# fanzhongyi/diffusion

Hardware: AMD Instinct MI355X
Metric: U-Net training images/sec @256 (SD-2-base U-Net, precomputed latents 4x32x32) (higher is better)
Workload: dtype bf16; 1 GPU; SD-2-base U-Net train step, latents 4x32x32, text 77x1024, batch 256/GPU (global 256), microbatch 256, AdamW, dp1; global_batch=256, microbatch=256, parallelism=dp1, params=865910724

## Files before the change

diffusion_amd/csrc/attention.hip:

```cpp
#include <type_traits>

#include "common.hpp"
#include "attn_lds.hpp"
#include "diffusion_amd.h"

namespace {

struct AttnParams {
  const bf16 *Q, *K, *V, *O, *dO;
  bf16 *Out, *dQ, *dK, *dV;
  float *L2, *Delta;
  long ldq, ldk, ldv, ldo, lddo, lddq, lddk, lddv;
  int B, H, Nq, Nk;
  float sc;
  float scale;
};

#ifdef DA_STAMPS
__device__ unsigned long long* g_attn_stamp_buf;
__device__ int g_attn_stamp_wgs;
#define ASTAMP(v) v = __builtin_amdgcn_s_memtime()
#else
#define ASTAMP(v) do {} while (0)
#endif

typedef float f32x2 __attribute__((ext_vector_type(2)));
DEVINL f32x2 pair(const f32x16& v, int i) { return f32x2{v[2 * i], v[2 * i + 1]}; }
DEVINL void set_pair(f32x16& v, int i, f32x2 x) { v[2 * i] = x.x; v[2 * i + 1] = x.y; }
DEVINL f32x2 fma2(f32x2 a, f32x2 b, f32x2 c) {
  float x = fmaf(a.x, b.x, c.x), y = fmaf(a.y, b.y, c.y);
  asm("" : "+v"(x));
  asm("" : "+v"(y));
  return f32x2{x, y};
}
DEVINL f32x2 mul2(f32x2 a, f32x2 b) {
  float x = a.x * b.x, y = a.y * b.y;
  asm("" : "+v"(x));
  asm("" : "+v"(y));
  return f32x2{x, y};
}
DEVINL f32x2 add2(f32x2 a, f32x2 b) {
  float x = a.x + b.x, y = a.y + b.y;
  asm("" : "+v"(x));
  asm("" : "+v"(y));
  return f32x2{x, y};
}
DEVINL f32x2 exp2_2(f32x2 x) { return f32x2{__builtin_amdgcn_exp2f(x.x), __builtin_amdgcn_exp2f(x.y)}; }

DEVINL float max3(float a, float b, float c) {
  float r;
  asm("v_max3_f32 %0, %1, %2, %3" : "=v"(r) : "v"(a), "v"(b), "v"(c));
  return r;
}

DEVINL void xcd_block_id(int& blk, int& hd, int& b) {
  const int nb = gridDim.x, nh = gridDim.y;
  const int total = nb * nh * gridDim.z;
  const int w = blockIdx.x + nb * (blockIdx.y + nh * blockIdx.z);
  const int q = total >> 3, r = total & 7;
// ... 8 lines not shown
__device__ __attribute__((aligned(256))) unsigned char g_attn_zero[256];
DEVINL void dma4(const void* g, char* l) {
  __builtin_amdgcn_global_load_lds((const __attribute__((address_space(1))) void*)g,
                                   (__attribute__((address_space(3))) void*)l, 4, 0, 0);
}

constexpr int FW_STAGE = 64 * 128 + 64 * TR_LD;

template <bool CAUSAL>
__global__ __launch_bounds__(256) void attn_fwd_kernel(AttnParams p) {
  extern __shared__ __attribute__((aligned(16))) char smem[];
  const int tid = threadIdx.x, lane = tid & 63;
  const int wave = __builtin_amdgcn_readfirstlane(tid >> 6);
  const int h = lane >> 5, r = lane & 31;
  int blk, hd, b;
  xcd_block_id(blk, hd, b);
  const int q = blk * 128 + wave * 32 + r;
  const bool qv = q < p.Nq;

  bf16x8 qf[4];
#pragma unroll
  for (int ks = 0; ks < 4; ++ks)
    qf[ks] = qv ? ld8(p.Q + ((long)b * p.Nq + q) * p.ldq + hd * 64 + ks * 16 + h * 8) : zero8();

  f32x16 o0, o1;
#pragma unroll
  for (int i = 0; i < 16; ++i) { o0[i] = 0.f; o1[i] = 0.f; }
  float m = -INFINITY, l = 0.f;

  const int nk_eff = CAUSAL ? min(p.Nk, blk * 128 + 128) : p.Nk;
  const int nt = (nk_eff + 63) / 64;
  const int drow = wave * 8 + (lane >> 3), pc = lane & 7;
  const int lc = (pc ^ swz_key(drow)) * 8;
  const bf16* kp = p.K + ((long)b * p.Nk + drow) * p.ldk + hd * 64;
  const bf16* vp = p.V + ((long)b * p.Nk + drow) * p.ldv + hd * 64;
  const char* zero = reinterpret_cast<const char*>(g_attn_zero);
  auto dma = [&](int t, int st) {
    char* S = smem + st * FW_STAGE + wave * 1024;
#pragma unroll
    for (int i = 0; i < 2; ++i) {
      const bool ok = t * 64 + drow + 32 * i < p.Nk;
      dma16(ok ? (const void*)(kp + 32 * i * p.ldk + lc) : (const void*)zero, S + i * 4096);
      dma16(ok ? (const void*)(vp + 32 * i * p.ldv + lc) : (const void*)zero, S + 8192 + i * 4096);
    }
    kp += 64 * p.ldk;
    vp += 64 * p.ldv;
  };
  auto sync_tile = [&]() {
    asm volatile("s_waitcnt vmcnt(0)" ::: "memory");
    __builtin_amdgcn_s_barrier();
    asm volatile("" ::: "memory");
  };

  dma(0, 0);
  sync_tile();
  auto step = [&](int t, auto tail_tag) {
    constexpr bool TAIL = decltype(tail_tag)::value;
    if (t + 1 < nt) dma(t + 1, (t + 1) & 1);
    const char* Ks = smem + (t & 1) * FW_STAGE;
    const char* Vs = Ks + 64 * 128;
    f32x16 s0, s1;
#pragma unroll
    for (int i = 0; i < 16; ++i) { s0[i] = 0.f; s1[i] = 0.f; }
#pragma unroll
    for (int ks = 0; ks < 4; ++ks) {
      bf16x8 k0 = *reinterpret_cast<const bf16x8*>(Ks + swz128(r, 2 * ks + h));
      bf16x8 k1 = *reinterpret_cast<const bf16x8*>(Ks + swz128(32 + r, 2 * ks + h));
      s0 = __builtin_amdgcn_mfma_f32_32x32x16_bf16(k0, qf[ks], s0, 0, 0, 0);
      s1 = __builtin_amdgcn_mfma_f32_32x32x16_bf16(k1, qf[ks], s1, 0, 0, 0);
    }
    short4v tv[2][4][2];
    const unsigned vto = lds_offset(Vs);
#pragma unroll
    for (int s2 = 0; s2 < 2; ++s2) {
      tr_frag_issue(vto, 16 * s2, 0, lane, tv[s2][0][0], tv[s2][0][1]);
      tr_frag_issue(vto, 16 * s2, 32, lane, tv[s2][1][0], tv[s2][1][1]);
      tr_frag_issue(vto, 32 + 16 * s2, 0, lane, tv[s2][2][0], tv[s2][2][1]);
      tr_frag_issue(vto, 32 + 16 * s2, 32, lane, tv[s2][3][0], tv[s2][3][1]);
    }
    if constexpr (TAIL) {
      const int klim = CAUSAL ? min(p.Nk, q + 1) : p.Nk;
#pragma unroll
      for (int i = 0; i < 16; ++i) {
        int key = t * 64 + acc_row(i, lane);
        if (key >= klim) s0[i] = -INFINITY;
        if (key + 32 >= klim) s1[i] = -INFINITY;
      }
    }
    float mx = fmaxf(s0[0], s1[0]);
#pragma unroll
    for (int i = 1; i < 16; ++i) mx = max3(mx, s0[i], s1[i]);
    mx = fmaxf(mx, xor32(mx));
    if (__any(mx > m)) {
      const float mn = fmaxf(m, mx);
      const float alpha = __builtin_amdgcn_exp2f((m - mn) * p.sc);
      l *= alpha;
      const f32x2 al2 = {alpha, alpha};
#pragma unroll
      for (int i = 0; i < 8; ++i) {
        set_pair(o0, i, mul2(pair(o0, i), al2));
        set_pair(o1, i, mul2(pair(o1, i), al2));
      }
      m = mn;
    }
    const float msc = -m * p.sc;
    const f32x2 sc2 = {p.sc, p.sc}, msc2 = {msc, msc};
    f32x2 ls2 = {0.f, 0.f};
#pragma unroll
    for (int i = 0; i < 8; ++i) {
      const f32x2 e0 = exp2_2(fma2(pair(s0, i), sc2, msc2));
      const f32x2 e1 = exp2_2(fma2(pair(s1, i), sc2, msc2));
      set_pair(s0, i, e0);
      set_pair(s1, i, e1);
      ls2 = add2(ls2, add2(e0, e1));
    }
    l += ls2.x + ls2.y;
    lds_wait_for<0>(tv[0][0][0], tv[0][0][1], tv[0][1][0], tv[0][1][1], tv[0][2][0], tv[0][2][1], tv[0][3][0], tv[0][3][1],
                    tv[1][0][0], tv[1][0][1], tv[1][1][0], tv[1][1][1], tv[1][2][0], tv[1][2][1], tv[1][3][0], tv[1][3][1]);
#pragma unroll
    for (int s2 = 0; s2 < 2; ++s2) {
      bf16x8 pa = pack8(s0, s2), pb = pack8(s1, s2);
      o0 = __builtin_amdgcn_mfma_f32_32x32x16_bf16(tr_frag_join(tv[s2][0][0], tv[s2][0][1]), pa, o0, 0, 0, 0);
      o1 = __builtin_amdgcn_mfma_f32_32x32x16_bf16(tr_frag_join(tv[s2][1][0], tv[s2][1][1]), pa, o1, 0, 0, 0);
      o0 = __builtin_amdgcn_mfma_f32_32x32x16_bf16(tr_frag_join(tv[s2][2][0], tv[s2][2][1]), pb, o0, 0, 0, 0);
      o1 = __builtin_amdgcn_mfma_f32_32x32x16_bf16(tr_frag_join(tv[s2][3][0], tv[s2][3][1]), pb, o1, 0, 0, 0);
    }
    sync_tile();
  };
  if constexpr (CAUSAL) {
    for (int t = 0; t < nt; ++t) step(t, std::true_type{});
  } else {
    const int nfull = p.Nk / 64;
    for (int t = 0; t < nfull; ++t) step(t, std::false_type{});
    if (nfull < nt) step(nfull, std::true_type{});
  }
  const float lt = l + xor32(l);
  const float inv = 1.0f / lt;
  if (qv) {
    bf16* op = p.Out + ((long)b * p.Nq + q) * p.ldo + hd * 64;
#pragma unroll
    for (int rg = 0; rg < 4; ++rg) {
      bf16x4 a, c;
#pragma unroll
      for (int e = 0; e < 4; ++e) {
        a[e] = f2bf(o0[rg * 4 + e] * inv);
        c[e] = f2bf(o1[rg * 4 + e] * inv);
      }
      *reinterpret_cast<bf16x4*>(op + 8 * rg + 4 * h) = a;
      *reinterpret_cast<bf16x4*>(op + 32 + 8 * rg + 4 * h) = c;
    }
    if (h == 0) p.L2[((long)b * p.H + hd) * p.Nq + q] = m * p.sc + log2f(lt);
  }
}

constexpr int DQ_STAGE = 2 * 64 * 128;

__global__ __launch_bounds__(256, 3) void attn_bwd_dq_kernel(AttnParams p) {
  extern __shared__ __attribute__((aligned(16))) char smem[];
  const int tid = threadIdx.x, lane = tid & 63;
  const int wave = __builtin_amdgcn_readfirstlane(tid >> 6);
  const int h = lane >> 5, r = lane & 31;
  int blk, hd, b;
  xcd_block_id(blk, hd, b);
  const int q = blk * 128 + wave * 32 + r;
  const bool qv = q < p.Nq;

  bf16x8 qf[4], dof[4];
  float delta = 0.f;
#pragma unroll
  for (int ks = 0; ks < 4; ++ks) {
    const int c = hd * 64 + ks * 16 + h * 8;
    qf[ks] = qv ? ld8(p.Q + ((long)b * p.Nq + q) * p.ldq + c) : zero8();
    dof[ks] = qv ? ld8(p.dO + ((long)b * p.Nq + q) * p.lddo + c) : zero8();
    bf16x8 of = qv ? ld8(p.O + ((long)b * p.Nq + q) * p.ldo + c) : zero8();
#pragma unroll
    for (int j = 0; j < 8; ++j) delta += bf2f(dof[ks][j]) * bf2f(of[j]);
  }
  delta += xor32(delta);
  const long statidx = ((long)b * p.H + hd) * p.Nq + q;
  const float nL2q = qv ? -p.L2[statidx] : 0.f;
  if (qv && h == 0) p.Delta[statidx] = delta;

  f32x16 d0, d1;
#pragma unroll
  for (int i = 0; i < 16; ++i) { d0[i] = 0.f; d1[i] = 0.f; }

  const int nt = (p.Nk + 63) / 64;
  const int drow = wave * 8 + (lane >> 3), pc = lane & 7;
  const int lc = (pc ^ swz_key(drow)) * 8;
  const bf16* kp = p.K + ((long)b * p.Nk + drow) * p.ldk + hd * 64;
  const bf16* vp = p.V + ((long)b * p.Nk + drow) * p.ldv + hd * 64;
  const char* zero = reinterpret_cast<const char*>(g_attn_zero);
  auto dma = [&](int t, int st) {
    char* S = smem + st * DQ_STAGE + wave * 1024;
#pragma unroll
    for (int i = 0; i < 2; ++i) {
      const bool ok = t * 64 + drow + 32 * i < p.Nk;
      dma16(ok ? (const void*)(kp + 32 * i * p.ldk + lc) : (const void*)zero, S + i * 4096);
      dma16(ok ? (const void*)(vp + 32 * i * p.ldv + lc) : (const void*)zero, S + 8192 + i * 4096);
    }
    kp += 64 * p.ldk;
    vp += 64 * p.ldv;
  };
  auto sync_tile = [&]() {
    asm volatile("s_waitcnt vmcnt(0)" ::: "memory");
    __builtin_amdgcn_s_barrier();
    asm volatile("" ::: "memory");
  };

  dma(0, 0);
  sync_tile();
  auto step = [&](int t, auto tail_tag) {
    constexpr bool TAIL = decltype(tail_tag)::value;
    if (t + 1 < nt) dma(t + 1, (t + 1) & 1);
    const char* Ks = smem + (t & 1) * DQ_STAGE;
    const char* Vs = Ks + 64 * 128;
    const char* Kt = Ks;
#pragma unroll
    for (int half = 0; half < 2; ++half) {
      const int kb = half * 32;
      if (TAIL && t * 64 + kb >= p.Nk) break;
      f32x16 s, dp;
#pragma unroll
      for (int i = 0; i < 16; ++i) { s[i] = 0.f; dp[i] = -delta; }
#pragma unroll
      for (int ks = 0; ks < 4; ++ks) {
        bf16x8 kf = *reinterpret_cast<const bf16x8*>(Ks + swz128(kb + r, 2 * ks + h));
        bf16x8 vf = *reinterpret_cast<const bf16x8*>(Vs + swz128(kb + r, 2 * ks + h));
        s = __builtin_amdgcn_mfma_f32_32x32x16_bf16(kf, qf[ks], s, 0, 0, 0);
        dp = __builtin_amdgcn_mfma_f32_32x32x16_bf16(vf, dof[ks], dp, 0, 0, 0);
      }
      short4v tk0[2][2], tk1[2][2];
      const unsigned kto = lds_offset(Kt);
#pragma unroll
      for (int s2 = 0; s2 < 2; ++s2) {
        tr_frag_issue(kto, kb + 16 * s2, 0, lane, tk0[s2][0], tk0[s2][1]);
        tr_frag_issue(kto, kb + 16 * s2, 32, lane, tk1[s2][0], tk1[s2][1]);
      }
      {
        const f32x2 sc2 = {p.sc, p.sc}, nl2 = {nL2q, nL2q};
#pragma unroll
        for (int i = 0; i < 8; ++i) {
          const f32x2 pv = exp2_2(__builtin_elementwise_fma(pair(s, i), sc2, nl2));
          set_pair(s, i, pv * pair(dp, i));
        }
      }
      if constexpr (TAIL) {
#pragma unroll
        for (int i = 0; i < 16; ++i)
          if (t * 64 + kb + acc_row(i, lane) >= p.Nk) s[i] = 0.f;
      }
      bf16x8 dsf[2] = {pack8(s, 0), pack8(s, 1)};
      lds_wait_for<0>(tk0[0][0], tk0[0][1], tk1[0][0], tk1[0][1], tk0[1][0], tk0[1][1], tk1[1][0], tk1[1][1]);
#pragma unroll
      for (int s2 = 0; s2 < 2; ++s2) {
        d0 = __builtin_amdgcn_mfma_f32_32x32x16_bf16(tr_frag_join(tk0[s2][0], tk0[s2][1]), dsf[s2], d0, 0, 0, 0);
        d1 = __builtin_amdgcn_mfma_f32_32x32x16_bf16(tr_frag_join(tk1[s2][0], tk1[s2][1]), dsf[s2], d1, 0, 0, 0);
      }
    }
    sync_tile();
  };
  const int nfull = p.Nk / 64;
  for (int t = 0; t < nfull; ++t) step(t, std::false_type{});
  if (nfull < nt) step(nfull, std::true_type{});
  if (qv) {
    bf16* op = p.dQ + ((long)b * p.Nq + q) * p.lddq + hd * 64;
#pragma unroll
    for (int rg = 0; rg < 4; ++rg) {
      bf16x4 a, c;
#pragma unroll
      for (int e = 0; e < 4; ++e) {
        a[e] = f2bf(d0[rg * 4 + e] * p.scale);
        c[e] = f2bf(d1[rg * 4 + e] * p.scale);
      }
      *reinterpret_cast<bf16x4*>(op + 8 * rg + 4 * h) = a;
      *reinterpret_cast<bf16x4*>(op + 32 + 8 * rg + 4 * h) = c;
    }
  }
}

constexpr int kv_stage(int QT) { return 2 * QT * 128 + 2 * QT * 4; }

template <int KV_QT>
__global__ __launch_bounds__(256, 2) void attn_bwd_dkv_kernel(AttnParams p) {
  constexpr int NW = 4, KV_SUB = KV_QT / 32, KV_STAGE = kv_stage(KV_QT);
  static_assert(KV_QT == 32 || KV_QT == 64, "query rows per tile");
  extern __shared__ __attribute__((aligned(16))) char smem[];
  const int tid = threadIdx.x, lane = tid & 63;
  const int wave = __builtin_amdgcn_readfirstlane(tid >> 6);
  const int h = lane >> 5, r = lane & 31;
  int blk, hd, b;
  xcd_block_id(blk, hd, b);
  const int key = blk * (32 * NW) + wave * 32 + r;
  const bool kv = key < p.Nk;

  bf16x8 kf[4], vf[4];
#pragma unroll
  for (int ks = 0; ks < 4; ++ks) {
    const int c = hd * 64 + ks * 16 + h * 8;
    kf[ks] = kv ? ld8(p.K + ((long)b * p.Nk + key) * p.ldk + c) : zero8();
    vf[ks] = kv ? ld8(p.V + ((long)b * p.Nk + key) * p.ldv + c) : zero8();
  }
  f32x16 dk0, dk1, dv0, dv1;
#pragma unroll
  for (int i = 0; i < 16; ++i) { dk0[i] = 0.f; dk1[i] = 0.f; dv0[i] = 0.f; dv1[i] = 0.f; }

  const int nt = (p.Nq + KV_QT - 1) / KV_QT;
  const int drow = (wave & 3) * 8 + (lane >> 3), pc = lane & 7;
  const int lc = (pc ^ swz_key(drow)) * 8;
  const bf16* qp = p.Q + ((long)b * p.Nq + drow) * p.ldq + hd * 64;
  const bf16* dop = p.dO + ((long)b * p.Nq + drow) * p.lddo + hd * 64;
  const float* statp = (lane < 32 ? p.L2 : p.Delta) + ((long)b * p.H + hd) * p.Nq + (lane & 31);
  const char* zero = reinterpret_cast<const char*>(g_attn_zero);
  auto dma = [&](int t, int st) {
    char* S = smem + st * KV_STAGE + (wave & 3) * 1024;
#pragma unroll
    for (int sub = 0; sub < KV_SUB; ++sub) {
      const bool ok = t * KV_QT + sub * 32 + drow < p.Nq;
      dma16(ok ? (const void*)(qp + sub * 32 * p.ldq + lc) : (const void*)zero, S + sub * 4096);
      dma16(ok ? (const void*)(dop + sub * 32 * p.lddo + lc) : (const void*)zero, S + KV_QT * 128 + sub * 4096);
      if (wave == 0) {
        const bool ok2 = t * KV_QT + sub * 32 + (lane & 31) < p.Nq;
        dma4(ok2 ? (const void*)(statp + sub * 32) : (const void*)zero, smem + st * KV_STAGE + 2 * KV_QT * 128 + sub * 256);
      }
    }
    qp += KV_QT * p.ldq;
    dop += KV_QT * p.lddo;
    statp += KV_QT;
  };
  auto sync_tiles = [&](bool newest_in_flight) {
    if (!newest_in_flight) asm volatile("s_waitcnt vmcnt(0)" ::: "memory");
    else if (wave == 0) asm volatile("s_waitcnt vmcnt(%0)" ::"n"(3 * KV_SUB) : "memory");
    else asm volatile("s_waitcnt vmcnt(%0)" ::"n"(2 * KV_SUB) : "memory");
    __builtin_amdgcn_s_barrier();
    asm volatile("" ::: "memory");
  };

  asm volatile("s_waitcnt vmcnt(0)" ::: "memory");
  dma(0, 0);
  if (nt > 1) dma(1, 1);
  sync_tiles(nt > 1);
  for (int t = 0; t < nt; ++t) {
#ifdef DA_STAMPS
    unsigned long long st0, st1, st2, st3, st4;
#endif
    ASTAMP(st0);
    if (t + 2 < nt) dma(t + 2, (t + 2) % 3);
#pragma unroll
    for (int sub = 0; sub < KV_SUB; ++sub) {
    const char* Qs = smem + (t % 3) * KV_STAGE + sub * 4096;
    const char* Os = Qs + KV_QT * 128;
    const char* Qt = Qs;
    const char* Ot = Os;
    const float* Ls = reinterpret_cast<const float*>(smem + (t % 3) * KV_STAGE + 2 * KV_QT * 128 + sub * 256);
    const float* Ds = Ls + 32;
    f32x16 s, dp;
#pragma unroll
    for (int rg = 0; rg < 4; ++rg) {
      const f32x4 d4 = *reinterpret_cast<const f32x4*>(Ds + 8 * rg + 4 * h);
#pragma unroll
      for (int e = 0; e < 4; ++e) { s[4 * rg + e] = 0.f; dp[4 * rg + e] = -d4[e]; }
    }
#pragma unroll
    for (int ks = 0; ks < 4; ++ks) {
      bf16x8 qf = *reinterpret_cast<const bf16x8*>(Qs + swz128(r, 2 * ks + h));
      bf16x8 of = *reinterpret_cast<const bf16x8*>(Os + swz128(r, 2 * ks + h));
      s = __builtin_amdgcn_mfma_f32_32x32x16_bf16(qf, kf[ks], s, 0, 0, 0);
      dp = __builtin_amdgcn_mfma_f32_32x32x16_bf16(of, vf[ks], dp, 0, 0, 0);
    }
    __builtin_amdgcn_sched_barrier(0);
    ASTAMP(st1);
    short4v to0[2][2], to1[2][2], tq0[2][2], tq1[2][2];
    const unsigned oto = lds_offset(Ot), qto = lds_offset(Qt);
#pragma unroll
    for (int s2 = 0; s2 < 2; ++s2) {
      tr_frag_issue(oto, 16 * s2, 0, lane, to0[s2][0], to0[s2][1]);
      tr_frag_issue(oto, 16 * s2, 32, lane, to1[s2][0], to1[s2][1]);
      tr_frag_issue(qto, 16 * s2, 0, lane, tq0[s2][0], tq0[s2][1]);
      tr_frag_issue(qto, 16 * s2, 32, lane, tq1[s2][0], tq1[s2][1]);
    }
    f32x16 pr;
#pragma unroll
    for (int rg = 0; rg < 4; ++rg) {
      const f32x4 l4 = *reinterpret_cast<const f32x4*>(Ls + 8 * rg + 4 * h);
      const f32x2 sc2 = {p.sc, p.sc};
#pragma unroll
      for (int e2 = 0; e2 < 2; ++e2) {
        const int i = rg * 2 + e2;
        const f32x2 pv = exp2_2(__builtin_elementwise_fma(pair(s, i), sc2, -f32x2{l4[2 * e2], l4[2 * e2 + 1]}));
        set_pair(pr, i, pv);
        set_pair(s, i, pv * pair(dp, i));
      }
    }
    bf16x8 pf[2] = {pack8(pr, 0), pack8(pr, 1)};
    bf16x8 dsf[2] = {pack8(s, 0), pack8(s, 1)};
    ASTAMP(st2);
    lds_wait_for<0>(to0[0][0], to0[0][1], to1[0][0], to1[0][1], tq0[0][0], tq0[0][1], tq1[0][0], tq1[0][1], to0[1][0],
                    to0[1][1], to1[1][0], to1[1][1], tq0[1][0], tq0[1][1], tq1[1][0], tq1[1][1]);
#pragma unroll
    for (int s2 = 0; s2 < 2; ++s2) {
      dv0 = __builtin_amdgcn_mfma_f32_32x32x16_bf16(tr_frag_join(to0[s2][0], to0[s2][1]), pf[s2], dv0, 0, 0, 0);
      dv1 = __builtin_amdgcn_mfma_f32_32x32x16_bf16(tr_frag_join(to1[s2][0], to1[s2][1]), pf[s2], dv1, 0, 0, 0);
      dk0 = __builtin_amdgcn_mfma_f32_32x32x16_bf16(tr_frag_join(tq0[s2][0], tq0[s2][1]), dsf[s2], dk0, 0, 0, 0);
      dk1 = __builtin_amdgcn_mfma_f32_32x32x16_bf16(tr_frag_join(tq1[s2][0], tq1[s2][1]), dsf[s2], dk1, 0, 0, 0);
    }
    }
    ASTAMP(st3);
    sync_tiles(t + 2 < nt);
    ASTAMP(st4);
#ifdef DA_STAMPS
    {
      const int wg = blockIdx.x + gridDim.x * (blockIdx.y + gridDim.y * blockIdx.z);
      if (g_attn_stamp_buf && wg < g_attn_stamp_wgs && (wave == 0 || wave == 3) && lane == 0 && t < 32) {
        unsigned long long* o = g_attn_stamp_buf + (((long)wg * 2 + (wave == 3)) * 32 + t) * 8;
        o[0] = st0; o[1] = st1; o[2] = st2; o[3] = st3; o[4] = st4;
      }
    }
#endif
  }
  if (kv) {
    bf16* kp = p.dK + ((long)b * p.Nk + key) * p.lddk + hd * 64;
    bf16* vp = p.dV + ((long)b * p.Nk + key) * p.lddv + hd * 64;
#pragma unroll
    for (int rg = 0; rg < 4; ++rg) {
      bf16x4 a, c, e0, e1;
#pragma unroll
      for (int e = 0; e < 4; ++e) {
        a[e] = f2bf(dk0[rg * 4 + e] * p.scale);
        c[e] = f2bf(dk1[rg * 4 + e] * p.scale);
        e0[e] = f2bf(dv0[rg * 4 + e]);
        e1[e] = f2bf(dv1[rg * 4 + e]);
      }
      *reinterpret_cast<bf16x4*>(kp + 8 * rg + 4 * h) = a;
      *reinterpret_cast<bf16x4*>(kp + 32 + 8 * rg + 4 * h) = c;
      *reinterpret_cast<bf16x4*>(vp + 8 * rg + 4 * h) = e0;
      *reinterpret_cast<bf16x4*>(vp + 32 + 8 * rg + 4 * h) = e1;
    }
  }
}

constexpr int FU_STAGE = 3 * 32 * 128 + 256;
constexpr int fu_ds(int NW) { return 32 * NW * 64; }
constexpr int fu_smem(int NW) { return 3 * FU_STAGE + 2 * fu_ds(NW) + NW * 128; }

template <int NW>
__global__ __launch_bounds__(64 * NW, 2) void attn_bwd_fused_kernel(AttnParams p) {
  constexpr int FU_DS = fu_ds(NW);
  constexpr int QTW = 8 / NW;
  extern __shared__ __attribute__((aligned(16))) char smem[];
  char* const dsbuf = smem + 3 * FU_STAGE;
  const int tid = threadIdx.x, lane = tid & 63;
  const int wave = __builtin_amdgcn_readfirstlane(tid >> 6);
  float* const dscr = reinterpret_cast<float*>(smem + 3 * FU_STAGE + 2 * FU_DS + wave * 128);
  const int h = lane >> 5, r = lane & 31;
  int blk, hd, b;
  xcd_block_id(blk, hd, b);
  const int key = wave * 32 + r;
  const bool kv = key < p.Nk;
  const int nkb = (p.Nk + 31) / 32;

  bf16x8 kf[4], vf[4];
#pragma unroll
  for (int ks = 0; ks < 4; ++ks) {
    const int c = hd * 64 + ks * 16 + h * 8;
    kf[ks] = kv ? ld8(p.K + ((long)b * p.Nk + key) * p.ldk + c) : zero8();
    vf[ks] = kv ? ld8(p.V + ((long)b * p.Nk + key) * p.ldv + c) : zero8();
  }
  {
    const int krow = tid >> 1, half = tid & 1;
    const bf16* src = p.K + ((long)b * p.Nk + krow) * p.ldk + hd * 64 + half * 32;
#pragma unroll
    for (int c = 0; c < 4; ++c) {
      const bf16x8 v = krow < p.Nk ? ld8(src + c * 8) : zero8();
      *reinterpret_cast<bf16x8*>(dsbuf + krow * 128 + half * 64 + c * 16) = v;
    }
  }
  __syncthreads();
  bf16x8 ktf[NW];
  const int dsl = wave & 3;
  {
    const int g = lane >> 4, i = lane & 15;
    const unsigned base = lds_offset(dsbuf) + (unsigned)((8 * g + (i >> 2)) * 128 + (16 * dsl + 4 * (i & 3)) * 2);
#pragma unroll
    for (int kb = 0; kb < NW; ++kb) {
      short4v t0 = lds_tr16_b64_asm(base + kb * 32 * 128);
      short4v t1 = lds_tr16_b64_asm(base + kb * 32 * 128 + 4 * 128);
      lds_wait_for<0>(t0, t1);
      ktf[kb] = tr_frag_join(t0, t1);
    }
  }
  __syncthreads();

  f32x16 dk0, dk1, dv0, dv1;
#pragma unroll
  for (int i = 0; i < 16; ++i) { dk0[i] = 0.f; dk1[i] = 0.f; dv0[i] = 0.f; dv1[i] = 0.f; }

  const int nt = (p.Nq + 31) / 32;
  const bool loader = wave < 4;
  const int drow = (wave & 3) * 8 + (lane >> 3), pc = lane & 7;
  const int lc = (pc ^ swz_key(drow)) * 8;
  const bf16* qp = p.Q + ((long)b * p.Nq + drow) * p.ldq + hd * 64;
  const bf16* dop = p.dO + ((long)b * p.Nq + drow) * p.lddo + hd * 64;
  const bf16* op = p.O + ((long)b * p.Nq + drow) * p.ldo + hd * 64;
  const long stat0 = ((long)b * p.H + hd) * p.Nq;
  const float* statp = p.L2 + stat0 + (lane & 31);
  const char* zero = reinterpret_cast<const char*>(g_attn_zero);
  auto dma = [&](int t, int st) {
    if (!loader) return;
    char* S = smem + st * FU_STAGE + wave * 1024;
    const bool ok = t * 32 + drow < p.Nq;
    dma16(ok ? (const void*)(qp + lc) : (const void*)zero, S);
    dma16(ok ? (const void*)(dop + lc) : (const void*)zero, S + 4096);
    dma16(ok ? (const void*)(op + lc) : (const void*)zero, S + 8192);
    if (wave == 0) {
      const bool ok2 = t * 32 + (lane & 31) < p.Nq;
      dma4(ok2 ? (const void*)statp : (const void*)zero, smem + st * FU_STAGE + 3 * 4096);
    }
    qp += 32 * p.ldq;
    dop += 32 * p.lddo;
    op += 32 * p.ldo;
    statp += 32;
  };
  auto sync_tiles = [&](bool newest_in_flight) {
    if (loader) {
      if (!newest_in_flight) asm volatile("s_waitcnt vmcnt(0)" ::: "memory");
      else if (wave == 0) asm volatile("s_waitcnt vmcnt(4)" ::: "memory");
      else asm volatile("s_waitcnt vmcnt(3)" ::: "memory");
    }
    __builtin_amdgcn_s_barrier();
    asm volatile("" ::: "memory");
  };
  auto dq_tile = [&](int t) {
    const int g = lane >> 4, i = lane & 15;
    const unsigned base = lds_offset(dsbuf + (t & 1) * FU_DS) + (unsigned)((8 * g + (i >> 2)) * 64 + (4 * (i & 3)) * 2);
    typedef float f32x4v __attribute__((ext_vector_type(4)));
#pragma unroll
    for (int qi = 0; qi < QTW; ++qi) {
      const int qt = (wave >> 2) * QTW + qi;
      f32x4v acc = {0.f, 0.f, 0.f, 0.f};
      short4v t0[NW], t1[NW];
#pragma unroll
      for (int kb = 0; kb < NW; ++kb) {
        t0[kb] = lds_tr16_b64_asm(base + kb * 32 * 64 + qt * 32);
        t1[kb] = lds_tr16_b64_asm(base + kb * 32 * 64 + qt * 32 + 4 * 64);
      }
#pragma unroll
      for (int kb = 0; kb < NW; ++kb) {
        lds_wait_for<0>(t0[kb], t1[kb]);
        if (kb < nkb) acc = __builtin_amdgcn_mfma_f32_16x16x32_bf16(ktf[kb], tr_frag_join(t0[kb], t1[kb]), acc, 0, 0, 0);
      }
      const int q = t * 32 + qt * 16 + i;
      if (q < p.Nq) {
        bf16x4 o;
#pragma unroll
        for (int e = 0; e < 4; ++e) o[e] = f2bf(acc[e] * p.scale);
        *reinterpret_cast<bf16x4*>(p.dQ + ((long)b * p.Nq + q) * p.lddq + hd * 64 + 16 * dsl + 4 * g) = o;
      }
    }
  };

  asm volatile("s_waitcnt vmcnt(0)" ::: "memory");
  dma(0, 0);
  if (nt > 1) dma(1, 1);
  sync_tiles(nt > 1);
  float delta_prev = 0.f;
  for (int t = 0; t < nt; ++t) {
    if (t > 0) {
      dq_tile(t - 1);
      if (wave == 0 && h == 0 && (t - 1) * 32 + r < p.Nq) p.Delta[stat0 + (t - 1) * 32 + r] = delta_prev;
    }
    if (t + 2 < nt) dma(t + 2, (t + 2) % 3);
    const char* Qs = smem + (t % 3) * FU_STAGE;
    const char* Os = Qs + 4096;
    const char* Oo = Qs + 8192;
    const float* Ls = reinterpret_cast<const float*>(Qs + 3 * 4096);
    bf16x8 of[4];
    float dpart = 0.f;
#pragma unroll
    for (int ks = 0; ks < 4; ++ks) {
      of[ks] = *reinterpret_cast<const bf16x8*>(Os + swz128(r, 2 * ks + h));
      const bf16x8 oo = *reinterpret_cast<const bf16x8*>(Oo + swz128(r, 2 * ks + h));
#pragma unroll
      for (int j = 0; j < 8; ++j) dpart = fmaf(bf2f(of[ks][j]), bf2f(oo[j]), dpart);
    }
    const float delta = dpart + xor32(dpart);
    if (h == 0) dscr[r] = delta;
    delta_prev = delta;
    asm volatile("s_waitcnt lgkmcnt(0)" ::: "memory");
    f32x16 s, dp;
#pragma unroll
    for (int rg = 0; rg < 4; ++rg) {
      const f32x4 d4 = *reinterpret_cast<const f32x4*>(dscr + 8 * rg + 4 * h);
#pragma unroll
      for (int e = 0; e < 4; ++e) { s[4 * rg + e] = 0.f; dp[4 * rg + e] = -d4[e]; }
    }
#pragma unroll
    for (int ks = 0; ks < 4; ++ks) {
      bf16x8 qf = *reinterpret_cast<const bf16x8*>(Qs + swz128(r, 2 * ks + h));
      s = __builtin_amdgcn_mfma_f32_32x32x16_bf16(qf, kf[ks], s, 0, 0, 0);
      dp = __builtin_amdgcn_mfma_f32_32x32x16_bf16(of[ks], vf[ks], dp, 0, 0, 0);
    }
    __builtin_amdgcn_sched_barrier(0);
    short4v to0[2][2], to1[2][2], tq0[2][2], tq1[2][2];
    const unsigned oto = lds_offset(Os), qto = lds_offset(Qs);
#pragma unroll
    for (int s2 = 0; s2 < 2; ++s2) {
      tr_frag_issue(oto, 16 * s2, 0, lane, to0[s2][0], to0[s2][1]);
      tr_frag_issue(oto, 16 * s2, 32, lane, to1[s2][0], to1[s2][1]);
      tr_frag_issue(qto, 16 * s2, 0, lane, tq0[s2][0], tq0[s2][1]);
      tr_frag_issue(qto, 16 * s2, 32, lane, tq1[s2][0], tq1[s2][1]);
    }
    f32x16 pr;
#pragma unroll
    for (int rg = 0; rg < 4; ++rg) {
      const f32x4 l4 = *reinterpret_cast<const f32x4*>(Ls + 8 * rg + 4 * h);
      const f32x2 sc2 = {p.sc, p.sc};
#pragma unroll
      for (int e2 = 0; e2 < 2; ++e2) {
        const int i = rg * 2 + e2;
        const f32x2 pv = exp2_2(__builtin_elementwise_fma(pair(s, i), sc2, -f32x2{l4[2 * e2], l4[2 * e2 + 1]}));
        set_pair(pr, i, pv);
        set_pair(s, i, pv * pair(dp, i));
      }
    }
    bf16x8 pf[2] = {pack8(pr, 0), pack8(pr, 1)};
    bf16x8 dsf[2] = {pack8(s, 0), pack8(s, 1)};
    if (!kv) { dsf[0] = zero8(); dsf[1] = zero8(); }
    {
      char* drow_p = dsbuf + (t & 1) * FU_DS + key * 64 + 8 * h;
      typedef __attribute__((ext_vector_type(4))) short short4w;
      typedef __attribute__((ext_vector_type(8))) short short8w;
#pragma unroll
      for (int s2 = 0; s2 < 2; ++s2) {
        const short8w v = __builtin_bit_cast(short8w, dsf[s2]);
        *reinterpret_cast<short4w*>(drow_p + 32 * s2) = __builtin_shufflevector(v, v, 0, 1, 2, 3);
        *reinterpret_cast<short4w*>(drow_p + 32 * s2 + 16) = __builtin_shufflevector(v, v, 4, 5, 6, 7);
      }
    }
    lds_wait_for<0>(to0[0][0], to0[0][1], to1[0][0], to1[0][1], tq0[0][0], tq0[0][1], tq1[0][0], tq1[0][1], to0[1][0],
                    to0[1][1], to1[1][0], to1[1][1], tq0[1][0], tq0[1][1], tq1[1][0], tq1[1][1]);
#pragma unroll
    for (int s2 = 0; s2 < 2; ++s2) {
      dv0 = __builtin_amdgcn_mfma_f32_32x32x16_bf16(tr_frag_join(to0[s2][0], to0[s2][1]), pf[s2], dv0, 0, 0, 0);
      dv1 = __builtin_amdgcn_mfma_f32_32x32x16_bf16(tr_frag_join(to1[s2][0], to1[s2][1]), pf[s2], dv1, 0, 0, 0);
      dk0 = __builtin_amdgcn_mfma_f32_32x32x16_bf16(tr_frag_join(tq0[s2][0], tq0[s2][1]), dsf[s2], dk0, 0, 0, 0);
      dk1 = __builtin_amdgcn_mfma_f32_32x32x16_bf16(tr_frag_join(tq1[s2][0], tq1[s2][1]), dsf[s2], dk1, 0, 0, 0);
    }
    asm volatile("s_waitcnt lgkmcnt(0)" ::: "memory");
    sync_tiles(t + 2 < nt);
  }
  dq_tile(nt - 1);
  if (wave == 0 && h == 0 && (nt - 1) * 32 + r < p.Nq) p.Delta[stat0 + (nt - 1) * 32 + r] = delta_prev;
  if (kv) {
    bf16* kp = p.dK + ((long)b * p.Nk + key) * p.lddk + hd * 64;
    bf16* vp = p.dV + ((long)b * p.Nk + key) * p.lddv + hd * 64;
#pragma unroll
    for (int rg = 0; rg < 4; ++rg) {
      bf16x4 a, c, e0, e1;
#pragma unroll
      for (int e = 0; e < 4; ++e) {
        a[e] = f2bf(dk0[rg * 4 + e] * p.scale);
        c[e] = f2bf(dk1[rg * 4 + e] * p.scale);
        e0[e] = f2bf(dv0[rg * 4 + e]);
        e1[e] = f2bf(dv1[rg * 4 + e]);
      }
      *reinterpret_cast<bf16x4*>(kp + 8 * rg + 4 * h) = a;
      *reinterpret_cast<bf16x4*>(kp + 32 + 8 * rg + 4 * h) = c;
      *reinterpret_cast<bf16x4*>(vp + 8 * rg + 4 * h) = e0;
      *reinterpret_cast<bf16x4*>(vp + 32 + 8 * rg + 4 * h) = e1;
    }
  }
}

int check(long ld) { return (ld & 7) ? 1 : 0; }

}

int g_attn_fused_bwd = 1;

#ifdef DA_STAMPS
extern "C" int da_debug_set_attn_stamps(void* buf, int wgs) {
  if (hipMemcpyToSymbol(HIP_SYMBOL(g_attn_stamp_buf), &buf, sizeof(buf)) != hipSuccess) return -1;
  return hipMemcpyToSymbol(HIP_SYMBOL(g_attn_stamp_wgs), &wgs, sizeof(wgs)) == hipSuccess ? 0 : -1;
}
#endif

extern "C" int da_attn_fwd(const void* Q, long ldq, const void* K, long ldk, const void* V, long ldv, void* O,
                           long ldo, float* L2, int B, int H, int Nq, int Nk, float scale, hipStream_t stream) {
  DA_CLEAR_ERR();
  if (B <= 0 || H <= 0 || Nq <= 0 || Nk <= 0) return DA_ERR_SHAPE;
  if (check(ldq) || check(ldk) || check(ldv) || check(ldo)) return DA_ERR_SHAPE;
  AttnParams p = {};
  p.Q = (const bf16*)Q; p.K = (const bf16*)K; p.V = (const bf16*)V; p.Out = (bf16*)O; p.L2 = L2;
  p.ldq = ldq; p.ldk = ldk; p.ldv = ldv; p.ldo = ldo;
  p.B = B; p.H = H; p.Nq = Nq; p.Nk = Nk;
  p.scale = scale; p.sc = scale * 1.4426950408889634f;
  hipLaunchKernelGGL(attn_fwd_kernel<false>, dim3((Nq + 127) / 128, H, B), dim3(256), 2 * FW_STAGE, stream, p);
  DA_CHECK_LAUNCH();
  return DA_OK;
}

extern "C" int da_attn_fwd_causal(const void* Q, long ldq, const void* K, long ldk, const void* V, long ldv, void* O,
                                  long ldo, float* L2, int B, int H, int N, float scale, hipStream_t stream) {
  DA_CLEAR_ERR();
// ... 52 lines not shown
```

diffusion_amd/csrc/attn_lds.hpp:

```cpp
#pragma once
#include "common.hpp"

namespace {

constexpr int TR_LD = 128;
DEVINL int swz_key(int row) { return (((row >> 1) & 1) << 2) | ((row >> 2) & 3); }
DEVINL int tr_off(int row, int bytecol) { return row * TR_LD + (bytecol ^ (swz_key(row) << 4)); }

DEVINL int swz128(int row, int chunk) { return row * 128 + ((chunk ^ swz_key(row)) << 4); }

DEVINL void tr_frag_issue(unsigned img_off, int row0, int col0, int lane, short4v& t0, short4v& t1) {
  const int gg = lane >> 4, dgrp = gg & 1, hh = gg >> 1, qq = (lane >> 2) & 3, pp = lane & 3;
  const int row = row0 + 4 * hh + qq, bc = (col0 + 16 * dgrp + 4 * pp) * 2;
  const unsigned a = img_off + tr_off(row, bc);
  t0 = lds_tr16_b64_asm(a);
  t1 = lds_tr16_b64_asm((a ^ 32u) + 8 * TR_LD);
}
DEVINL bf16x8 tr_frag_join(short4v t0, short4v t1) {
  typedef __attribute__((ext_vector_type(8))) short short8v;
  short8v v = __builtin_shufflevector(t0, t1, 0, 1, 2, 3, 4, 5, 6, 7);
  return __builtin_bit_cast(bf16x8, v);
}

DEVINL bf16x8 pack8(const f32x16& x, int s) {
  bf16x8 r;
#pragma unroll
  for (int j = 0; j < 8; ++j) r[j] = f2bf(x[8 * s + j]);
  return r;
}

DEVINL void dma16(const void* g, char* l) {
  __builtin_amdgcn_global_load_lds((const __attribute__((address_space(1))) void*)g,
                                   (__attribute__((address_space(3))) void*)l, 16, 0, 0);
}

DEVINL int acc_row(int reg, int lane) { return (reg & 3) + 8 * (reg >> 2) + 4 * (lane >> 5); }

}
```

diffusion_amd/csrc/common.hpp:

```cpp
#pragma once
#include <hip/hip_runtime.h>
#include <stdint.h>

typedef __bf16 bf16;
typedef __attribute__((ext_vector_type(8))) __bf16 bf16x8;
typedef __attribute__((ext_vector_type(4))) __bf16 bf16x4;
typedef __attribute__((ext_vector_type(2))) __bf16 bf16x2;
typedef __attribute__((ext_vector_type(4))) short short4v;
typedef __attribute__((ext_vector_type(4))) float f32x4;
typedef __attribute__((ext_vector_type(16))) float f32x16;
typedef __attribute__((ext_vector_type(4))) unsigned int u32x4;

#define DEVINL __device__ __forceinline__

#define DA_OK 0
#define DA_ERR_SHAPE 1
#define DA_ERR_LAUNCH 2

#define DA_CLEAR_ERR() (void)hipGetLastError()

#define DA_CHECK_LAUNCH()                                   \
  do {                                                      \
    hipError_t e__ = hipGetLastError();                     \
    if (e__ != hipSuccess) return DA_ERR_LAUNCH;            \
// ... 61 lines not shown
  return __builtin_amdgcn_rcpf(1.0f + __builtin_amdgcn_exp2f(-1.4426950408889634f * x));
}
DEVINL float silu_f(float x) { return x * sigmoid_f(x); }
DEVINL float dsilu_f(float x) {
  const float s = sigmoid_f(x);
  return s * fmaf(x, 1.0f - s, 1.0f);
}
DEVINL float gelu_phi(float x, float& e) {
  const float z = fabsf(x) * 0.70710678118654752f;
  const float t = __builtin_amdgcn_rcpf(fmaf(0.3275911f, z, 1.0f));
  float poly = fmaf(1.061405429f, t, -1.453152027f);
  poly = fmaf(poly, t, 1.421413741f);
  poly = fmaf(poly, t, -0.284496736f);
  poly = fmaf(poly, t, 0.254829592f);
  poly *= t;
  e = __builtin_amdgcn_exp2f(-(z * z) * 1.4426950408889634f);
  const float er = copysignf(fmaf(-poly, e, 1.0f), x);
  return fmaf(0.5f, er, 0.5f);
}
DEVINL float gelu_f(float x) {
  float e;
  return x * gelu_phi(x, e);
}
DEVINL float dgelu_f(float x) {
  float e;
  const float cdf = gelu_phi(x, e);
  return fmaf(x * 0.39894228040143268f, e, cdf);
}

struct FastDiv {
  unsigned long long magic;
  unsigned int d;
};
DEVINL unsigned int fdiv(unsigned int n, FastDiv f) { return (unsigned int)(((unsigned long long)n * f.magic) >> 40); }
static inline FastDiv make_fastdiv(unsigned int d) {
  FastDiv f;
  f.d = d;
  f.magic = ((1ull << 40) / d) + 1ull;
  return f;
}

DEVINL short4v lds_tr16_b64(const void* lds_addr) {
  return __builtin_amdgcn_ds_read_tr16_b64_v4i16((__attribute__((address_space(3))) short4v*)(lds_addr));
}

DEVINL unsigned lds_offset(const void* p) {
  return (unsigned)(unsigned long)(const __attribute__((address_space(3))) char*)p;
}
DEVINL short4v lds_tr16_b64_asm(unsigned lds_byte_offset) {
  short4v r;
  asm volatile("ds_read_b64_tr_b16 %0, %1" : "=v"(r) : "v"(lds_byte_offset));
  return r;
}
template <int N>
DEVINL void lds_wait() {
  asm volatile("s_waitcnt lgkmcnt(%0)" ::"n"(N) : "memory");
}
template <typename T>
DEVINL void reg_tie(T& r) {
  asm volatile("" : "+v"(r));
}
template <int N, typename... T>
DEVINL void lds_wait_for(T&... regs) {
  asm volatile("s_waitcnt lgkmcnt(%0)" ::"n"(N) : "memory");
  (reg_tie(regs), ...);
}
```

Baseline: 1564 images/sec.

## Precompute LDS offsets and unroll attention loops by stage for immediate addressing

Per-lane swizzled LDS row offsets and transpose-read base addresses are computed once outside the tile loops and pinned in registers. The loops are unrolled by pipeline stage (2 or 3) so stage offsets become compile-time immediates in the ds_read offset field, removing per-iteration address arithmetic. The fused backward kernel also gets a third dS buffer with an XOR-swizzled layout to reduce bank conflicts, and skips compute for waves with no keys. The cost is more LDS, larger code and extra pinned VGPRs, which could lower occupancy.

Result: no change. 1568 images/sec (median of 6 runs) (+0.3%).

```diff
diff --git a/diffusion_amd/csrc/attention.hip b/diffusion_amd/csrc/attention.hip
--- a/diffusion_amd/csrc/attention.hip
+++ b/diffusion_amd/csrc/attention.hip
@@ -5,6 +5,9 @@
 #include "diffusion_amd.h"
 
 namespace {
+
+template <int N>
+using ic = std::integral_constant<int, N>;
 
 struct AttnParams {
   const bf16 *Q, *K, *V, *O, *dO;
@@ -119,31 +122,37 @@
     asm volatile("" ::: "memory");
   };
 
+  int kro[4];
+  unsigned vto[4];
+  row_offs(r, h, kro);
+  tr_offs(lds_offset(smem), lane, vto);
+
   dma(0, 0);
   sync_tile();
-  auto step = [&](int t, auto tail_tag) {
+#pragma unroll
+  for (int ks = 0; ks < 4; ++ks) asm volatile("" ::"v"(qf[ks]));
+  auto step = [&](int t, const int (&kro)[4], const unsigned (&vto)[4], auto st_tag, auto tail_tag) {
+    constexpr int ST = decltype(st_tag)::value;
     constexpr bool TAIL = decltype(tail_tag)::value;
-    if (t + 1 < nt) dma(t + 1, (t + 1) & 1);
-    const char* Ks = smem + (t & 1) * FW_STAGE;
-    const char* Vs = Ks + 64 * 128;
+    if (t + 1 < nt) dma(t + 1, ST ^ 1);
+    constexpr int KS = ST * FW_STAGE, VS = KS + 64 * 128;
     f32x16 s0, s1;
 #pragma unroll
     for (int i = 0; i < 16; ++i) { s0[i] = 0.f; s1[i] = 0.f; }
 #pragma unroll
     for (int ks = 0; ks < 4; ++ks) {
-      bf16x8 k0 = *reinterpret_cast<const bf16x8*>(Ks + swz128(r, 2 * ks + h));
-      bf16x8 k1 = *reinterpret_cast<const bf16x8*>(Ks + swz128(32 + r, 2 * ks + h));
+      bf16x8 k0 = *reinterpret_cast<const bf16x8*>(smem + (kro[ks] + KS));
+      bf16x8 k1 = *reinterpret_cast<const bf16x8*>(smem + (kro[ks] + (KS + 32 * 128)));
       s0 = __builtin_amdgcn_mfma_f32_32x32x16_bf16(k0, qf[ks], s0, 0, 0, 0);
       s1 = __builtin_amdgcn_mfma_f32_32x32x16_bf16(k1, qf[ks], s1, 0, 0, 0);
     }
     short4v tv[2][4][2];
-    const unsigned vto = lds_offset(Vs);
 #pragma unroll
     for (int s2 = 0; s2 < 2; ++s2) {
-      tr_frag_issue(vto, 16 * s2, 0, lane, tv[s2][0][0], tv[s2][0][1]);
-      tr_frag_issue(vto, 16 * s2, 32, lane, tv[s2][1][0], tv[s2][1][1]);
-      tr_frag_issue(vto, 32 + 16 * s2, 0, lane, tv[s2][2][0], tv[s2][2][1]);
-      tr_frag_issue(vto, 32 + 16 * s2, 32, lane, tv[s2][3][0], tv[s2][3][1]);
+      tr_frag_issue_at(vto, 0, VS + 16 * s2 * TR_LD, tv[s2][0][0], tv[s2][0][1]);
+      tr_frag_issue_at(vto, 1, VS + 16 * s2 * TR_LD, tv[s2][1][0], tv[s2][1][1]);
+      tr_frag_issue_at(vto, 0, VS + (32 + 16 * s2) * TR_LD, tv[s2][2][0], tv[s2][2][1]);
+      tr_frag_issue_at(vto, 1, VS + (32 + 16 * s2) * TR_LD, tv[s2][3][0], tv[s2][3][1]);
     }
     if constexpr (TAIL) {
       const int klim = CAUSAL ? min(p.Nk, q + 1) : p.Nk;
@@ -195,11 +204,26 @@
     sync_tile();
   };
   if constexpr (CAUSAL) {
-    for (int t = 0; t < nt; ++t) step(t, std::true_type{});
+    for (int t = 0; t < nt; t += 2) {
+      step(t, kro, vto, ic<0>{}, std::true_type{});
+      if (t + 1 < nt) step(t + 1, kro, vto, ic<1>{}, std::true_type{});
+    }
   } else {
     const int nfull = p.Nk / 64;
-    for (int t = 0; t < nfull; ++t) step(t, std::false_type{});
-    if (nfull < nt) step(nfull, std::true_type{});
+    for (int t = 0; t < nfull; t += 2) {
+      step(t, kro, vto, ic<0>{}, std::false_type{});
+      if (t + 1 < nfull) step(t + 1, kro, vto, ic<1>{}, std::false_type{});
+    }
+    if (nfull < nt) {
+      int krt[4];
+      unsigned vtt[4];
+#pragma unroll
+      for (int j = 0; j < 4; ++j) {
+        krt[j] = kro[j] + (nfull & 1) * FW_STAGE;
+        vtt[j] = vto[j] + (unsigned)((nfull & 1) * FW_STAGE);
+      }
+      step(nfull, krt, vtt, ic<0>{}, std::true_type{});
+    }
   }
   const float lt = l + xor32(l);
   const float inv = 1.0f / lt;
@@ -275,14 +299,19 @@
     asm volatile("" ::: "memory");
   };
 
+  unsigned kto[4];
+  tr_offs(lds_offset(smem), lane, kto);
+
   dma(0, 0);
   sync_tile();
   auto step = [&](int t, auto tail_tag) {
     constexpr bool TAIL = decltype(tail_tag)::value;
     if (t + 1 < nt) dma(t + 1, (t + 1) & 1);
     const char* Ks = smem + (t & 1) * DQ_STAGE;
+    unsigned kts[4];
+#pragma unroll
+    for (int j = 0; j < 4; ++j) kts[j] = kto[j] + (unsigned)((t & 1) * DQ_STAGE);
     const char* Vs = Ks + 64 * 128;
-    const char* Kt = Ks;
 #pragma unroll
     for (int half = 0; half < 2; ++half) {
       const int kb = half * 32;
@@ -298,11 +327,10 @@
         dp = __builtin_amdgcn_mfma_f32_32x32x16_bf16(vf, dof[ks], dp, 0, 0, 0);
       }
       short4v tk0[2][2], tk1[2][2];
-      const unsigned kto = lds_offset(Kt);
 #pragma unroll
       for (int s2 = 0; s2 < 2; ++s2) {
-        tr_frag_issue(kto, kb + 16 * s2, 0, lane, tk0[s2][0], tk0[s2][1]);
-        tr_frag_issue(kto, kb + 16 * s2, 32, lane, tk1[s2][0], tk1[s2][1]);
+        tr_frag_issue_at(kts, 0, (kb + 16 * s2) * TR_LD, tk0[s2][0], tk0[s2][1]);
+        tr_frag_issue_at(kts, 1, (kb + 16 * s2) * TR_LD, tk1[s2][0], tk1[s2][1]);
       }
       {
         const f32x2 sc2 = {p.sc, p.sc}, nl2 = {nL2q, nL2q};
@@ -403,23 +431,26 @@
     asm volatile("" ::: "memory");
   };
 
+  int qro[4];
+  unsigned qto[4];
+  row_offs(r, h, qro);
+  tr_offs(lds_offset(smem), lane, qto);
+
   asm volatile("s_waitcnt vmcnt(0)" ::: "memory");
   dma(0, 0);
   if (nt > 1) dma(1, 1);
   sync_tiles(nt > 1);
-  for (int t = 0; t < nt; ++t) {
+  auto tile = [&](int t, auto st_tag) {
+    constexpr int ST = decltype(st_tag)::value;
 #ifdef DA_STAMPS
     unsigned long long st0, st1, st2, st3, st4;
 #endif
     ASTAMP(st0);
-    if (t + 2 < nt) dma(t + 2, (t + 2) % 3);
+    if (t + 2 < nt) dma(t + 2, (ST + 2) % 3);
 #pragma unroll
     for (int sub = 0; sub < KV_SUB; ++sub) {
-    const char* Qs = smem + (t % 3) * KV_STAGE + sub * 4096;
-    const char* Os = Qs + KV_QT * 128;
-    const char* Qt = Qs;
-    const char* Ot = Os;
-    const float* Ls = reinterpret_cast<const float*>(smem + (t % 3) * KV_STAGE + 2 * KV_QT * 128 + sub * 256);
+    const int QS = ST * KV_STAGE + sub * 4096, OS = QS + KV_QT * 128;
+    const float* Ls = reinterpret_cast<const float*>(smem + ST * KV_STAGE + 2 * KV_QT * 128 + sub * 256);
     const float* Ds = Ls + 32;
     f32x16 s, dp;
 #pragma unroll
@@ -430,21 +461,20 @@
     }
 #pragma unroll
     for (int ks = 0; ks < 4; ++ks) {
-      bf16x8 qf = *reinterpret_cast<const bf16x8*>(Qs + swz128(r, 2 * ks + h));
-      bf16x8 of = *reinterpret_cast<const bf16x8*>(Os + swz128(r, 2 * ks + h));
+      bf16x8 qf = *reinterpret_cast<const bf16x8*>(smem + (qro[ks] + QS));
+      bf16x8 of = *reinterpret_cast<const bf16x8*>(smem + (qro[ks] + OS));
       s = __builtin_amdgcn_mfma_f32_32x32x16_bf16(qf, kf[ks], s, 0, 0, 0);
       dp = __builtin_amdgcn_mfma_f32_32x32x16_bf16(of, vf[ks], dp, 0, 0, 0);
     }
     __builtin_amdgcn_sched_barrier(0);
     ASTAMP(st1);
     short4v to0[2][2], to1[2][2], tq0[2][2], tq1[2][2];
-    const unsigned oto = lds_offset(Ot), qto = lds_offset(Qt);
 #pragma unroll
     for (int s2 = 0; s2 < 2; ++s2) {
-      tr_frag_issue(oto, 16 * s2, 0, lane, to0[s2][0], to0[s2][1]);
-      tr_frag_issue(oto, 16 * s2, 32, lane, to1[s2][0], to1[s2][1]);
-      tr_frag_issue(qto, 16 * s2, 0, lane, tq0[s2][0], tq0[s2][1]);
-      tr_frag_issue(qto, 16 * s2, 32, lane, tq1[s2][0], tq1[s2][1]);
+      tr_frag_issue_at(qto, 0, OS + 16 * s2 * TR_LD, to0[s2][0], to0[s2][1]);
+      tr_frag_issue_at(qto, 1, OS + 16 * s2 * TR_LD, to1[s2][0], to1[s2][1]);
+      tr_frag_issue_at(qto, 0, QS + 16 * s2 * TR_LD, tq0[s2][0], tq0[s2][1]);
+      tr_frag_issue_at(qto, 1, QS + 16 * s2 * TR_LD, tq1[s2][0], tq1[s2][1]);
     }
     f32x16 pr;
 #pragma unroll
@@ -484,6 +514,13 @@
       }
     }
 #endif
+  };
+  for (int t = 0; t < nt; t += 3) {
+    tile(t, ic<0>{});
+    if (t + 1 < nt) {
+      tile(t + 1, ic<1>{});
+      if (t + 2 < nt) tile(t + 2, ic<2>{});
+    }
   }
   if (kv) {
     bf16* kp = p.dK + ((long)b * p.Nk + key) * p.lddk + hd * 64;
@@ -508,7 +545,8 @@
 
 constexpr int FU_STAGE = 3 * 32 * 128 + 256;
 constexpr int fu_ds(int NW) { return 32 * NW * 64; }
-constexpr int fu_smem(int NW) { return 3 * FU_STAGE + 2 * fu_ds(NW) + NW * 128; }
+constexpr int fu_smem(int NW) { return 3 * FU_STAGE + 3 * fu_ds(NW) + NW * 128; }
+DEVINL int ds_key(int key) { return ((key >> 1) & 4) | ((key >> 3) & 2) | ((key >> 2) & 1); }
 
 template <int NW>
 __global__ __launch_bounds__(64 * NW, 2) void attn_bwd_fused_kernel(AttnParams p) {
@@ -518,7 +556,7 @@
   char* const dsbuf = smem + 3 * FU_STAGE;
   const int tid = threadIdx.x, lane = tid & 63;
   const int wave = __builtin_amdgcn_readfirstlane(tid >> 6);
-  float* const dscr = reinterpret_cast<float*>(smem + 3 * FU_STAGE + 2 * FU_DS + wave * 128);
+  float* const dscr = reinterpret_cast<float*>(smem + 3 * FU_STAGE + 3 * FU_DS + wave * 128);
   const int h = lane >> 5, r = lane & 31;
   int blk, hd, b;
   xcd_block_id(blk, hd, b);
@@ -597,9 +635,31 @@
     __builtin_amdgcn_s_barrier();
     asm volatile("" ::: "memory");
   };
-  auto dq_tile = [&](int t) {
+  int qro[4];
+  unsigned qto[4];
+  row_offs(r, h, qro);
+  tr_offs(lds_offset(smem), lane, qto);
+  int dso[4];
+#pragma unroll
+  for (int rg = 0; rg < 4; ++rg) {
+    dso[rg] = key * 64 + 8 * ((2 * rg + h) ^ ds_key(key));
+    pin(dso[rg]);
+  }
+  unsigned dsr[2 * QTW];
+  {
+    const int g = lane >> 4, i = lane & 15, row = 8 * g + (i >> 2);
+#pragma unroll
+    for (int qi = 0; qi < QTW; ++qi)
+#pragma unroll
+      for (int e = 0; e < 2; ++e) {
+        const int qt = (wave >> 2) * QTW + qi;
+        dsr[2 * qi + e] = lds_offset(dsbuf) + (unsigned)(row * 64 + 8 * ((4 * qt + (i & 3)) ^ ds_key(row) ^ e));
+        pin(dsr[2 * qi + e]);
+      }
+  }
+  auto dq_tile = [&](int t, const unsigned (&rd)[2 * QTW], auto img_tag) {
+    constexpr int IMG = decltype(img_tag)::value;
     const int g = lane >> 4, i = lane & 15;
-    const unsigned base = lds_offset(dsbuf + (t & 1) * FU_DS) + (unsigned)((8 * g + (i >> 2)) * 64 + (4 * (i & 3)) * 2);
     typedef float f32x4v __attribute__((ext_vector_type(4)));
 #pragma unroll
     for (int qi = 0; qi < QTW; ++qi) {
@@ -608,8 +668,8 @@
       short4v t0[NW], t1[NW];
 #pragma unroll
       for (int kb = 0; kb < NW; ++kb) {
-        t0[kb] = lds_tr16_b64_asm(base + kb * 32 * 64 + qt * 32);
-        t1[kb] = lds_tr16_b64_asm(base + kb * 32 * 64 + qt * 32 + 4 * 64);
+        t0[kb] = lds_tr16_b64_asm(rd[2 * qi], IMG + kb * 32 * 64);
+        t1[kb] = lds_tr16_b64_asm(rd[2 * qi + 1], IMG + kb * 32 * 64 + 4 * 64);
       }
 #pragma unroll
       for (int kb = 0; kb < NW; ++kb) {
@@ -631,22 +691,23 @@
   if (nt > 1) dma(1, 1);
   sync_tiles(nt > 1);
   float delta_prev = 0.f;
-  for (int t = 0; t < nt; ++t) {
+  const bool has_keys = wave * 32 < p.Nk;
+  auto tile = [&](int t, auto st_tag) {
+    constexpr int ST = decltype(st_tag)::value;
     if (t > 0) {
-      dq_tile(t - 1);
+      dq_tile(t - 1, dsr, ic<((ST + 2) % 3) * FU_DS>{});
       if (wave == 0 && h == 0 && (t - 1) * 32 + r < p.Nq) p.Delta[stat0 + (t - 1) * 32 + r] = delta_prev;
     }
-    if (t + 2 < nt) dma(t + 2, (t + 2) % 3);
-    const char* Qs = smem + (t % 3) * FU_STAGE;
-    const char* Os = Qs + 4096;
-    const char* Oo = Qs + 8192;
-    const float* Ls = reinterpret_cast<const float*>(Qs + 3 * 4096);
+    if (t + 2 < nt) dma(t + 2, (ST + 2) % 3);
+    if (has_keys) {
+    constexpr int QS = ST * FU_STAGE, OS = QS + 4096, OO = QS + 8192;
+    const float* Ls = reinterpret_cast<const float*>(smem + QS + 3 * 4096);
     bf16x8 of[4];
     float dpart = 0.f;
 #pragma unroll
     for (int ks = 0; ks < 4; ++ks) {
-      of[ks] = *reinterpret_cast<const bf16x8*>(Os + swz128(r, 2 * ks + h));
-      const bf16x8 oo = *reinterpret_cast<const bf16x8*>(Oo + swz128(r, 2 * ks + h));
+      of[ks] = *reinterpret_cast<const bf16x8*>(smem + (qro[ks] + OS));
+      const bf16x8 oo = *reinterpret_cast<const bf16x8*>(smem + (qro[ks] + OO));
 #pragma unroll
       for (int j = 0; j < 8; ++j) dpart = fmaf(bf2f(of[ks][j]), bf2f(oo[j]), dpart);
     }
@@ -663,19 +724,18 @@
     }
 #pragma unroll
     for (int ks = 0; ks < 4; ++ks) {
-      bf16x8 qf = *reinterpret_cast<const bf16x8*>(Qs + swz128(r, 2 * ks + h));
+      bf16x8 qf = *reinterpret_cast<const bf16x8*>(smem + (qro[ks] + QS));
       s = __builtin_amdgcn_mfma_f32_32x32x16_bf16(qf, kf[ks], s, 0, 0, 0);
       dp = __builtin_amdgcn_mfma_f32_32x32x16_bf16(of[ks], vf[ks], dp, 0, 0, 0);
     }
     __builtin_amdgcn_sched_barrier(0);
     short4v to0[2][2], to1[2][2], tq0[2][2], tq1[2][2];
-    const unsigned oto = lds_offset(Os), qto = lds_offset(Qs);
 #pragma unroll
     for (int s2 = 0; s2 < 2; ++s2) {
-      tr_frag_issue(oto, 16 * s2, 0, lane, to0[s2][0], to0[s2][1]);
-      tr_frag_issue(oto, 16 * s2, 32, lane, to1[s2][0], to1[s2][1]);
-      tr_frag_issue(qto, 16 * s2, 0, lane, tq0[s2][0], tq0[s2][1]);
-      tr_frag_issue(qto, 16 * s2, 32, lane, tq1[s2][0], tq1[s2][1]);
+      tr_frag_issue_at(qto, 0, OS + 16 * s2 * TR_LD, to0[s2][0], to0[s2][1]);
+      tr_frag_issue_at(qto, 1, OS + 16 * s2 * TR_LD, to1[s2][0], to1[s2][1]);
+      tr_frag_issue_at(qto, 0, QS + 16 * s2 * TR_LD, tq0[s2][0], tq0[s2][1]);
+      tr_frag_issue_at(qto, 1, QS + 16 * s2 * TR_LD, tq1[s2][0], tq1[s2][1]);
     }
     f32x16 pr;
 #pragma unroll
@@ -694,14 +754,13 @@
     bf16x8 dsf[2] = {pack8(s, 0), pack8(s, 1)};
     if (!kv) { dsf[0] = zero8(); dsf[1] = zero8(); }
     {
-      char* drow_p = dsbuf + (t & 1) * FU_DS + key * 64 + 8 * h;
       typedef __attribute__((ext_vector_type(4))) short short4w;
       typedef __attribute__((ext_vector_type(8))) short short8w;
 #pragma unroll
       for (int s2 = 0; s2 < 2; ++s2) {
         const short8w v = __builtin_bit_cast(short8w, dsf[s2]);
-        *reinterpret_cast<short4w*>(drow_p + 32 * s2) = __builtin_shufflevector(v, v, 0, 1, 2, 3);
-        *reinterpret_cast<short4w*>(drow_p + 32 * s2 + 16) = __builtin_shufflevector(v, v, 4, 5, 6, 7);
+        *reinterpret_cast<short4w*>(dsbuf + (dso[2 * s2] + ST * FU_DS)) = __builtin_shufflevector(v, v, 0, 1, 2, 3);
+        *reinterpret_cast<short4w*>(dsbuf + (dso[2 * s2 + 1] + ST * FU_DS)) = __builtin_shufflevector(v, v, 4, 5, 6, 7);
       }
     }
     lds_wait_for<0>(to0[0][0], to0[0][1], to1[0][0], to1[0][1], tq0[0][0], tq0[0][1], tq1[0][0], tq1[0][1], to0[1][0],
@@ -714,9 +773,22 @@
       dk1 = __builtin_amdgcn_mfma_f32_32x32x16_bf16(tr_frag_join(tq1[s2][0], tq1[s2][1]), dsf[s2], dk1, 0, 0, 0);
     }
     asm volatile("s_waitcnt lgkmcnt(0)" ::: "memory");
+    }
     sync_tiles(t + 2 < nt);
-  }
-  dq_tile(nt - 1);
+  };
+  for (int t = 0; t < nt; t += 3) {
+    tile(t, ic<0>{});
+    if (t + 1 < nt) {
+      tile(t + 1, ic<1>{});
+      if (t + 2 < nt) tile(t + 2, ic<2>{});
+    }
+  }
+  {
+    unsigned dsl_[2 * QTW];
+#pragma unroll
+    for (int j = 0; j < 2 * QTW; ++j) dsl_[j] = dsr[j] + (unsigned)(((nt - 1) % 3) * FU_DS);
+    dq_tile(nt - 1, dsl_, ic<0>{});
+  }
   if (wave == 0 && h == 0 && (nt - 1) * 32 + r < p.Nq) p.Delta[stat0 + (nt - 1) * 32 + r] = delta_prev;
   if (kv) {
     bf16* kp = p.dK + ((long)b * p.Nk + key) * p.lddk + hd * 64;
diff --git a/diffusion_amd/csrc/attn_lds.hpp b/diffusion_amd/csrc/attn_lds.hpp
--- a/diffusion_amd/csrc/attn_lds.hpp
+++ b/diffusion_amd/csrc/attn_lds.hpp
@@ -15,6 +15,28 @@
   const unsigned a = img_off + tr_off(row, bc);
   t0 = lds_tr16_b64_asm(a);
   t1 = lds_tr16_b64_asm((a ^ 32u) + 8 * TR_LD);
+}
+DEVINL void pin(int& x) { asm("" : "+v"(x)); }
+DEVINL void pin(unsigned& x) { asm("" : "+v"(x)); }
+DEVINL void row_offs(int row, int h, int (&o)[4]) {
+#pragma unroll
+  for (int ks = 0; ks < 4; ++ks) {
+    o[ks] = swz128(row, 2 * ks + h);
+    pin(o[ks]);
+  }
+}
+DEVINL void tr_offs(unsigned base, int lane, unsigned (&o)[4]) {
+  const int gg = lane >> 4, dgrp = gg & 1, hh = gg >> 1, qq = (lane >> 2) & 3, pp = lane & 3;
+  const unsigned a = tr_off(4 * hh + qq, (16 * dgrp + 4 * pp) * 2);
+#pragma unroll
+  for (int j = 0; j < 4; ++j) {
+    o[j] = base + (a ^ (32u * j));
+    pin(o[j]);
+  }
+}
+DEVINL void tr_frag_issue_at(const unsigned (&o)[4], int c, int imm, short4v& t0, short4v& t1) {
+  t0 = lds_tr16_b64_asm(o[2 * c], imm);
+  t1 = lds_tr16_b64_asm(o[2 * c + 1], imm + 8 * TR_LD);
 }
 DEVINL bf16x8 tr_frag_join(short4v t0, short4v t1) {
   typedef __attribute__((ext_vector_type(8))) short short8v;
diff --git a/diffusion_amd/csrc/common.hpp b/diffusion_amd/csrc/common.hpp
--- a/diffusion_amd/csrc/common.hpp
+++ b/diffusion_amd/csrc/common.hpp
@@ -137,6 +137,11 @@
   asm volatile("ds_read_b64_tr_b16 %0, %1" : "=v"(r) : "v"(lds_byte_offset));
   return r;
 }
+DEVINL short4v lds_tr16_b64_asm(unsigned lds_byte_offset, int imm) {
+  short4v r;
+  asm volatile("ds_read_b64_tr_b16 %0, %1 offset:%2" : "=v"(r) : "v"(lds_byte_offset), "i"(imm));
+  return r;
+}
 template <int N>
 DEVINL void lds_wait() {
   asm volatile("s_waitcnt lgkmcnt(%0)" ::"n"(N) : "memory");
```
